# aconverse/ffmpeg-heaac

Measured on AMD Instinct MI355X. Metric: HE-AAC frames/s (batched), higher is better.
Workload: dtype f32; 1 GPU; HE-AACv2 stereo 48 kHz, 256 k-frame batch; frames_per_gpu=262144, pcm=f32, bytes_per_frame=85284, parallelism=frames sharded by index, no collective

## Files before the change

### ffmpeg-heaac_amd/__init__.py

```python
import ctypes as C
import os

import numpy as np

_HERE = os.path.dirname(os.path.abspath(__file__))
PRODUCT_LIB_PATH = os.path.join(_HERE, "libheaac_amd.so")
LIB_PATH = os.environ.get("HEAAC_LIB_PATH") or PRODUCT_LIB_PATH
LIB_OVERRIDDEN = os.path.realpath(LIB_PATH) != os.path.realpath(PRODUCT_LIB_PATH)

ONLY_LONG_SEQUENCE, LONG_START_SEQUENCE, EIGHT_SHORT_SEQUENCE, LONG_STOP_SEQUENCE = 0, 1, 2, 3
CFG_LC_MONO, CFG_LC_STEREO, CFG_HEV1, CFG_HEV2, CFG_HEV1_MONO = 0, 1, 2, 3, 4
PCM_F32, PCM_S16, PCM_S16_SSE2 = 0, 1, 2
ADD_BIAS = 385.0

ST_SAVED, ST_SBR, ST_SYNTH, ST_PS = 512, 1972, 1152, 4500
STATE_WORDS = {
    CFG_LC_MONO: ST_SAVED,
    CFG_LC_STEREO: 2 * ST_SAVED,
    CFG_HEV1: 2 * ST_SAVED + 2 * ST_SBR + 2 * ST_SYNTH,
    CFG_HEV1_MONO: ST_SAVED + ST_SBR + ST_SYNTH,
    CFG_HEV2: ST_SAVED + ST_SBR + 2 * ST_SYNTH + ST_PS,
}
CORE_CH = {CFG_LC_MONO: 1, CFG_LC_STEREO: 2, CFG_HEV1: 2, CFG_HEV2: 1, CFG_HEV1_MONO: 1}
OUT_CH = {CFG_LC_MONO: 1, CFG_LC_STEREO: 2, CFG_HEV1: 2, CFG_HEV2: 2, CFG_HEV1_MONO: 1}
OUT_LEN = {CFG_LC_MONO: 1024, CFG_LC_STEREO: 1024, CFG_HEV1: 2048, CFG_HEV2: 2048, CFG_HEV1_MONO: 2048}

ALGO_BYTES = {CFG_LC_STEREO: 24584, CFG_HEV1: 83976, CFG_HEV2: 85284}

ICS_DT = np.dtype([("window_sequence", "u1", (2,)), ("use_kb_window", "u1", (2,))])
SBR_HDR_DT = np.dtype([
    ("k0", "u1"), ("k2", "u1"), ("kx", "u1"), ("m", "u1"),
    ("n", "u1", (2,)), ("n_q", "u1"), ("n_lim", "u1"),
    ("n_master", "u1"), ("num_patches", "u1"), ("bs_limiter_gains", "u1"),
    ("bs_interpol_freq", "u1"), ("bs_smoothing_mode", "u1"), ("bs_amp_res_header", "u1"),
    ("pad0", "u1", (2,)),
    ("patch_num_subbands", "u1", (6,)), ("patch_start_subband", "u1", (6,)),
    ("f_tablenoise", "u1", (6,)), ("pad1", "u1", (2,)),
    ("f_tablelow", "u1", (28,)), ("f_tablehigh", "u1", (52,)), ("f_tablelim", "u1", (32,)),
    ("map_hi", "u1", (64,)), ("map_lo", "u1", (64,)), ("map_nq", "u1", (64,)),
    ("map_lim", "u1", (64,)), ("map_mid", "u1", (64,)), ("map_src", "u1", (64,)),
])
SBR_CH_DT = np.dtype([
    ("bs_num_env", "u1"), ("bs_num_noise", "u1"), ("bs_amp_res", "u1"), ("bs_add_harmonic_flag", "u1"),
    ("bs_freq_res", "u1", (8,)), ("t_env", "u1", (8,)), ("t_q", "u1", (3,)),
    ("t_env_num_env_old", "u1"), ("e_a", "i1", (2,)),
    ("bs_invf_mode", "u1", (2, 5)), ("bs_add_harmonic", "u1", (48,)),
# ... 1121 lines not shown
```

### ffmpeg-heaac_amd/csrc/capi.hip

```cpp
#include <hip/hip_runtime.h>
#include <stdint.h>
#include <stdlib.h>
#include <string.h>
#include "heaac_dsp.h"
#include "heaac_debug.h"
#include "heaac_parse.h"
#include "parse_core.h"
#include "sbr_core.h"
#include "tables.h"
#include "kernels.h"
#include "host_common.h"

#define HE_MAX_LANES 4
#define HE_ZERO_BYTES (2 * 38 * 64 * 4)
struct HeaacDevice {
    int device;
    float *d_tab;
    uint16_t *d_rev;
    HeaacParseTables *d_ptab;
    HeaacSbrParseTables *d_stab;
    void *d_work;
    unsigned *d_queue;
    unsigned char *d_aux;
    size_t work_bytes;
    size_t max_frames;
    size_t chunk;
    int sets;
    hipStream_t lane[HE_MAX_LANES];
    hipEvent_t fork, join[HE_MAX_LANES];
    int lanes;
    hipStream_t owner;
    hipEvent_t done;
    int owner_valid, done_recorded;
};

static int he_claim(HeaacDevice *d, hipStream_t s, bool *capturing)
{
// ... 88 lines not shown
    *out = NULL;
    int count = 0;
    if (hipGetDeviceCount(&count) != hipSuccess || count <= 0)
        return HEAAC_ERR_NODEVICE;
    HeaacDevice *d = (HeaacDevice *)calloc(1, sizeof(*d));
    if (!d) return HEAAC_ERR_NOMEM;
    if (hipGetDevice(&d->device) != hipSuccess) { free(d); return HEAAC_ERR_HIP; }
    hipDeviceProp_t prop;
    if (hipGetDeviceProperties(&prop, d->device) != hipSuccess ||
        strncmp(prop.gcnArchName, "gfx950", 6) != 0) {
        free(d);
        return HEAAC_ERR_NODEVICE;
    }
    HeaacHostTables *t = (HeaacHostTables *)malloc(sizeof(*t));
    if (!t) { free(d); return HEAAC_ERR_NOMEM; }
    heaac_build_tables(t);
    d->max_frames = max_frames;
    d->work_bytes = heaac_device_workspace_bytes(max_frames);
    d->chunk = he_chunk_frames(max_frames);
    d->sets = (int)he_sets(max_frames);
    int rc = HEAAC_OK;
    if (hipMalloc((void **)&d->d_tab, sizeof(t->f)) != hipSuccess ||
        hipMalloc((void **)&d->d_rev, sizeof(t->rev)) != hipSuccess ||
        hipMalloc((void **)&d->d_queue, 64 * HE_MAX_LANES) != hipSuccess ||
        hipMalloc((void **)&d->d_aux, HE_ZERO_BYTES + 2 * (size_t)(d->sets > 0 ? d->sets : 1) * (d->chunk ? d->chunk : 1)) != hipSuccess ||
        hipMalloc((void **)&d->d_ptab, sizeof(HeaacParseTables)) != hipSuccess ||
        hipMalloc((void **)&d->d_stab, sizeof(HeaacSbrParseTables)) != hipSuccess ||
        (d->work_bytes && hipMalloc(&d->d_work, d->work_bytes) != hipSuccess))
        rc = HEAAC_ERR_NOMEM;
    const HeaacParseTables *pt = heaac_parse_tables();
    if (rc == HEAAC_OK && (!pt || hipMemcpy(d->d_ptab, pt, sizeof(*pt), hipMemcpyHostToDevice) != hipSuccess))
        rc = HEAAC_ERR_HIP;
    const HeaacSbrParseTables *spt = heaac_sbr_parse_tables();
    if (rc == HEAAC_OK && (!spt || hipMemcpy(d->d_stab, spt, sizeof(*spt), hipMemcpyHostToDevice) != hipSuccess))
        rc = HEAAC_ERR_HIP;
    if (rc == HEAAC_OK &&
        (hipMemset(d->d_aux, 0, HE_ZERO_BYTES) != hipSuccess ||
         hipMemcpy(d->d_tab, t->f, sizeof(t->f), hipMemcpyHostToDevice) != hipSuccess ||
         hipMemcpy(d->d_rev, t->rev, sizeof(t->rev), hipMemcpyHostToDevice) != hipSuccess))
        rc = HEAAC_ERR_HIP;
    free(t);
    d->lanes = HE_LANES;
    if (rc == HEAAC_OK && (hipEventCreateWithFlags(&d->fork, hipEventDisableTiming) != hipSuccess ||
                           hipEventCreateWithFlags(&d->done, hipEventDisableTiming) != hipSuccess))
        rc = HEAAC_ERR_HIP;
    for (int k = 0; k < d->lanes && rc == HEAAC_OK; k++)
        if (hipEventCreateWithFlags(&d->join[k], hipEventDisableTiming) != hipSuccess ||
            hipStreamCreateWithFlags(&d->lane[k], hipStreamNonBlocking) != hipSuccess)
            rc = HEAAC_ERR_HIP;
    if (rc != HEAAC_OK) {
        heaac_device_destroy(d);
        return rc;
    }
    *out = d;
    return HEAAC_OK;
}

extern "C" void heaac_device_destroy(HeaacDevice *d)
{
    if (!d) return;
    if (d->d_tab) (void)hipFree(d->d_tab);
// ... 235 lines not shown
    const HeaacCfgShape shape = heaac_cfg_shape(cfg);
    const size_t ncore = shape.ncore, words = shape.words;
    const size_t pcm_bytes = (size_t)shape.nout * ((flags & HEAAC_HE_DOWNSAMPLED) ? 1024 : 2048) *
                             (pcm_format == HEAAC_PCM_F32_PLANAR ? 4 : 2);
    const size_t set_floats = dev->chunk * (WS_W_FLOATS + WS_X_FLOATS);
    const size_t per_chunk = dev->chunk / T;
    const unsigned hdrs = (unsigned)(n_hdr > 0xffffu ? 0x10000u : n_hdr);
    bool capturing = false;
    const int claim = he_claim(dev, s, &capturing);
    if (claim != HEAAC_OK) return claim;
    const bool lanes = n_streams > per_chunk && dev->sets > 1;
    const int nl = lanes ? dev->sets : 1;
    int rc = HEAAC_OK;
    int forked = 0;
    if (lanes) {
        if (hipEventRecord(dev->fork, s) != hipSuccess) rc = HEAAC_ERR_HIP;
        for (int k = 0; k < nl && rc == HEAAC_OK; k++) {
            if (hipStreamWaitEvent(dev->lane[k], dev->fork, 0) != hipSuccess) rc = HEAAC_ERR_HIP;
            else forked = k + 1;
        }
    }
    HeaacHeLaunch a = {};
    a.d_tab = dev->d_tab; a.d_rev = dev->d_rev; a.cfg = cfg; a.flags = flags; a.d_hdr = d_hdr; a.n_hdr = hdrs;
    a.pcm_format = pcm_format; a.d_zero = (const float *)dev->d_aux; a.T = T;
    size_t c = 0;
    for (size_t s0 = 0; s0 < n_streams && rc == HEAAC_OK; s0 += per_chunk, c++) {
        const size_t f0 = s0 * T;
        const int k = (int)(c % nl);
        a.n_streams = n_streams - s0 < per_chunk ? n_streams - s0 : per_chunk;
        a.d_coeffs = d_coeffs + f0 * ncore * 1024; a.d_ics = d_ics + f0 * ncore; a.d_sbr = d_sbr + f0;
        a.d_ps = d_ps ? d_ps + f0 : NULL; a.d_hold = d_hold ? d_hold + f0 : NULL;
        a.d_state_in = d_state_in + s0 * words; a.d_state_out = d_state_out + s0 * words;
        a.d_pcm = (char *)d_pcm + f0 * pcm_bytes;
        a.d_ws_W = (float *)dev->d_work + k * set_floats; a.d_ws_X = a.d_ws_W + dev->chunk * WS_W_FLOATS;
        a.d_queue = dev->d_queue + 16 * k; a.d_xtop = dev->d_aux + HE_ZERO_BYTES + 2 * (size_t)k * dev->chunk;
        a.s = lanes ? dev->lane[k] : s;
        rc = heaac_launch_he(&a);
    }
    if (lanes) {
        for (int k = 0; k < forked; k++)
            if (hipEventRecord(dev->join[k], dev->lane[k]) != hipSuccess ||
                hipStreamWaitEvent(s, dev->join[k], 0) != hipSuccess)
                rc = rc == HEAAC_OK ? HEAAC_ERR_HIP : rc;
    }
    return he_release(dev, s, capturing, rc);
}

extern "C" int heaac_he_decode_batch_ex(HeaacDevice *dev, int cfg, int flags,
                                     const float *d_coeffs, const HeaacIcs *d_ics,
                                     const HeaacSbrFrame *d_sbr,
                                     const HeaacSbrHeader *d_hdr, size_t n_hdr,
                                     const HeaacPsFrame *d_ps,
                                     const float *d_state_in, float *d_state_out,
                                     void *d_pcm, int pcm_format,
                                     size_t n, void *stream)
{
    if (!dev || !he_cfg_ok(cfg) || !pcm_format_ok(pcm_format) || (flags & ~HEAAC_HE_DOWNSAMPLED))
        return HEAAC_ERR_ARG;
// ... 105 lines not shown
    if (!dev || channels < 1 || channels > HEAAC_MAX_PCM_PLANES || len <= 0 || (len & 3) ||
        (pcm_format != HEAAC_PCM_S16_INTERLEAVED && pcm_format != HEAAC_PCM_S16_INTERLEAVED_SSE2))
        return HEAAC_ERR_ARG;
    if (n == 0) return HEAAC_OK;
    if (!planes || !d_out) return HEAAC_ERR_ARG;
    for (int c = 0; c < channels; c++)
        if (!planes[c].d_base || ((uintptr_t)planes[c].d_base & 15) || (planes[c].frame_stride & 3)) return HEAAC_ERR_ARG;
    return heaac_launch_interleave(channels, planes, len, pcm_format, d_out, n, (hipStream_t)stream);
}

extern "C" int heaac_debug_workspace(HeaacDevice *dev, float **d_W, float **d_X, size_t *chunk)
{
    if (!dev) return HEAAC_ERR_ARG;
    if (d_W) *d_W = (float *)dev->d_work;
    if (d_X) *d_X = (float *)dev->d_work + dev->chunk * WS_W_FLOATS;
    if (chunk) *chunk = dev->chunk;
    return HEAAC_OK;
}

extern "C" int heaac_debug_xbands(HeaacDevice *dev, unsigned char *host_out, size_t n_frames)
{
    if (!dev || !host_out || n_frames > (size_t)(dev->sets > 0 ? dev->sets : 1) * dev->chunk) return HEAAC_ERR_ARG;
    if (hipDeviceSynchronize() != hipSuccess) return HEAAC_ERR_HIP;
    return hipMemcpy(host_out, dev->d_aux + HE_ZERO_BYTES, 2 * n_frames, hipMemcpyDeviceToHost) == hipSuccess
               ? HEAAC_OK : HEAAC_ERR_HIP;
}

size_t heaac_device_max_frames_per_stream(const HeaacDevice *dev) { return dev ? dev->chunk : 0; }

extern "C" const float *heaac_device_tables(HeaacDevice *dev, const uint16_t **rev)
{
    if (rev) *rev = dev->d_rev;
    return dev->d_tab;
}
```

### ffmpeg-heaac_amd/csrc/k_common.h

```cpp
#pragma once
#include <hip/hip_runtime.h>
#include "heaac_dsp.h"
#include <stdint.h>
#include <type_traits>
#include "tables.h"

#define WAVE 64

__device__ __forceinline__ void wave_sync()
{
    __builtin_amdgcn_fence(__ATOMIC_RELEASE, "wavefront");
    __builtin_amdgcn_wave_barrier();
    __builtin_amdgcn_fence(__ATOMIC_ACQUIRE, "wavefront");
}

typedef float v2f __attribute__((ext_vector_type(2)));

__device__ __forceinline__ const uint8_t *hold_mask() { return nullptr; }
__device__ __forceinline__ const uint8_t *hold_mask(const uint8_t *p) { return p; }

#define HE_X_CHANNEL (38 * 64 * 2)

template <int ST_AUX>
struct GBufT {
// ... 55 lines not shown
        qoff = waves * Q;
        pos = 0;
        cur = wave * Q;
        unsigned t = 0;
        if (lane == 0) t = atomicAdd(queue, Q);
        base1 = qoff + (unsigned long long)__builtin_amdgcn_readfirstlane(t);
        nxt = Q > 1 ? cur + 1 : base1;
        vt = 0;
    }
    __device__ __forceinline__ void request(int lane)
    {
        if (pos == 0) { vt = 0; if (lane == 0) vt = atomicAdd(queue, Q); }
    }
    __device__ __forceinline__ void advance()
    {
        cur = nxt;
        if (pos + 1 < Q) {
            pos++;
        } else {
            pos = 0;
            base1 = qoff + (unsigned long long)__builtin_amdgcn_readfirstlane(vt);
        }
        nxt = pos + 1 < Q ? cur + 1 : base1;
    }
};

struct NoHook {
    __device__ __forceinline__ void operator()() const {}
    __device__ __forceinline__ void operator()(int) const {}
};

__device__ __forceinline__ unsigned lds_addr(const void *p)
{
    return __builtin_amdgcn_readfirstlane((unsigned)reinterpret_cast<uintptr_t>(p));
}
#define L2_TOUCH_STRIDE 128
__device__ __forceinline__ void l2_touch(const void *base, unsigned bytes, int lane, unsigned dump)
{
    for (unsigned o = 0; o < bytes; o += WAVE * L2_TOUCH_STRIDE) {
        unsigned off = o + (unsigned)lane * L2_TOUCH_STRIDE;
        off = off < bytes ? off : bytes - 4;
        const char *p = reinterpret_cast<const char *>(base) + off;
        unsigned keep;
        asm volatile("s_mov_b32 %0, m0\n\ts_mov_b32 m0, %2\n\ts_nop 0\n\t"
                     "global_load_lds_dword %1, off\n\ts_mov_b32 m0, %0"
                     : "=&s"(keep) : "v"(p), "s"(dump) : "memory");
// ... 236 lines not shown
```

### ffmpeg-heaac_amd/csrc/k_he.hip

```cpp
#include <type_traits>
#include "k_core.h"
#include "k_core2.h"
#include "kernels.h"
#include "host_common.h"

#include "k_hf.h"

#define ANA_WAVES 8
#define ANA_POOL  3456

struct AnaLds {
    CoreLds core;
    float qmf_ds[320];
    float rot[64];
    float pool[ANA_WAVES][ANA_POOL];
};

__device__ __forceinline__ void qmf_analysis_wave(const float *qmf_ds, const float *rot,
                                                  const float *c16, const float *c32,
                                                  const float *x, float *u, float *g_W, int lane)
{
    {
        const int k = lane;
        const float w0 = qmf_ds[k], w1 = qmf_ds[k + 64], w2 = qmf_ds[k + 128],
// ... 238 lines not shown
        int xb = 64;
        hf_channel(S, s_noise, sbr, g_hdr, n_hdr, ch, g_W + u * 2048,
                   g_state_in + f * state_words + off, g_state_out + f * state_words + off, lane,
                   [&](int i, float re, float im) {
                       if (i == 0 && g_xtop) {
                           const int top16 = (S.h.kx + S.h.m + 15) & ~15;
                           const int t_old = S.c[ch].t_env_num_env_old;
                           const bool zero = 2 * t_old - 32 <= 0 || (int)sbr->kx_old + (int)sbr->m_old <= top16;
                           xb = __builtin_amdgcn_readfirstlane(zero && top16 < 64 ? top16 : 64);
                           if (lane == 0 && xb != 64) g_xtop[f * 2 + ch] = (unsigned char)xb;
                       }
                       if (lane < xb) __builtin_nontemporal_store(v2f{re, im}, Xc + i * 64 + lane);
                   });
      }
        feed.advance();
    }
}

#define SYN_WAVES 6
#define VB_STRIDE 129
#define VB_ROWS   41

#define SYN_WAVES_F32 7
struct SynWave {
    __attribute__((aligned(16))) float vb[VB_ROWS * VB_STRIDE + 3];
};
template <int NW>
struct SynLdsT {
    float win[640];
    float rot[64];
    float c16[8], c32[12];
    SynWave w[NW];
};
typedef SynLdsT<SYN_WAVES> SynLds;

#ifdef HEAAC_STAMPS
#define SSTAMP(i) TL_STAMP(i, (i) == 0)
#else
#define SSTAMP(i) do {} while (0)
#endif

__device__ __forceinline__ float lane_xor1(float v)
{
    return __int_as_float(__builtin_amdgcn_update_dpp(0, __float_as_int(v), 0xB1, 0xF, 0xF, false));
}

struct SynIn {
    float x[64];
    float h[18];
};

#define SYN_STAGE_STRIDE 68
typedef float f32x4 __attribute__((ext_vector_type(4)));
__device__ __forceinline__ f32x4 syn_ld4(const f32x4 *p) { return __builtin_nontemporal_load(p); }
__device__ __forceinline__ float syn_ld1(const float *p) { return __builtin_nontemporal_load(p); }
template <class T>
__device__ __forceinline__ void syn_st(T *p, T v) { __builtin_nontemporal_store(v, p); }
__device__ __forceinline__ void syn_load_ring(const float *v_in, int lane, SynIn &d)
{
#pragma unroll
    for (int r = 0; r < 18; r++) d.h[r] = syn_ld1(v_in + lane + 64 * r);
}
template <bool PLANES, bool RING = true>
__device__ __forceinline__ void syn_load(const float *X0, const float *X1, const float *v_in, int lane, SynIn &d)
{
    const f32x4 *p0 = reinterpret_cast<const f32x4 *>(X0), *p1 = reinterpret_cast<const f32x4 *>(X1);
#pragma unroll
    for (int q = 0; q < 16; q++) {
        const f32x4 t = PLANES ? syn_ld4(q < 8 ? p0 + q * 64 + lane : p1 + (q - 8) * 64 + lane)
                               : syn_ld4(p0 + q * 64 + lane);
        d.x[4 * q] = t.x; d.x[4 * q + 1] = t.y; d.x[4 * q + 2] = t.z; d.x[4 * q + 3] = t.w;
    }
    if constexpr (RING) syn_load_ring(v_in, lane, d);
}

template <bool PLANES, class SL>
__device__ __forceinline__ void syn_rows(const SL &S, SynWave &w, const SynIn &d, int lane)
{
    float x[64];
    {
        float4 *st = reinterpret_cast<float4 *>(w.vb);
        if constexpr (PLANES) {
#pragma unroll
            for (int q = 0; q < 16; q++) {
                const int row = (q >> 3) * 32 + 4 * (q & 7) + (lane >> 4);
                st[(row * SYN_STAGE_STRIDE >> 2) + (lane & 15)] = make_float4(d.x[4 * q], d.x[4 * q + 1], d.x[4 * q + 2], d.x[4 * q + 3]);
            }
        } else {
            float2 *st2 = reinterpret_cast<float2 *>(w.vb);
#pragma unroll
            for (int q = 0; q < 16; q++) {
                const int slot = 2 * q + (lane >> 5), pi = lane & 31;
                st2[(slot * SYN_STAGE_STRIDE >> 1) + pi] = make_float2(d.x[4 * q], d.x[4 * q + 2]);
                st2[((32 + slot) * SYN_STAGE_STRIDE >> 1) + pi] = make_float2(d.x[4 * q + 1], d.x[4 * q + 3]);
            }
        }
        wave_sync();
        const int mine = (lane & 1) * 32 + (lane >> 1);
#pragma unroll
        for (int q = 0; q < 16; q++) {
            const float4 t = st[(mine * SYN_STAGE_STRIDE >> 2) + q];
            x[4 * q] = t.x; x[4 * q + 1] = t.y; x[4 * q + 2] = t.z; x[4 * q + 3] = t.w;
        }
        wave_sync();
    }
    SSTAMP(1);
#pragma unroll
    for (int r = 0; r < 18; r++)
        w.vb[(32 + (r >> 1)) * VB_STRIDE + (r & 1) * 64 + lane] = d.h[r];
    const int i = lane >> 1, part = lane & 1;
    const unsigned flip = (unsigned)part << 31;
    float o[64];
    imdct128_reg([&](int j) -> float {
                     return (j & 1) ? __uint_as_float(__float_as_uint(x[j]) ^ flip) : x[j];
                 }, o, S.rot, S.c16, S.c32);
    SSTAMP(2);
    float *vs = w.vb + (31 - i) * VB_STRIDE + 64 * part;
    const unsigned neg = (unsigned)(part ^ 1) << 31;
#pragma unroll
    for (int n = 0; n < 64; n++) {
        const float mine = __uint_as_float(__float_as_uint(o[63 - n]) ^ neg);
        vs[n] = lane_xor1(o[n]) + mine;
    }
}

template <int UNROLL = 1, class SL, class Emit>
__device__ __forceinline__ void syn_poly(const SL &S, const SynWave &w, float scale, float bias, int lane, Emit emit)
{
    SSTAMP(3);
    const int n = lane;
    float wt[10];
#pragma unroll
    for (int j = 0; j < 10; j++) wt[j] = S.win[64 * j + n];
    const bool scale_and_bias = scale != 1.0f || bias != 0.0f;
#pragma unroll UNROLL
    for (int i = 0; i < 32; i += 2) {
        const float *va = w.vb + (31 - i) * VB_STRIDE + n, *vb = va - VB_STRIDE;
        v2f acc = v2f{va[0], vb[0]} * bc(wt[0]) + v2f{0.0f, 0.0f};
        acc = v2f{va[1 * VB_STRIDE + 64], vb[1 * VB_STRIDE + 64]} * bc(wt[1]) + acc;
        acc = v2f{va[2 * VB_STRIDE],      vb[2 * VB_STRIDE]}      * bc(wt[2]) + acc;
        acc = v2f{va[3 * VB_STRIDE + 64], vb[3 * VB_STRIDE + 64]} * bc(wt[3]) + acc;
        acc = v2f{va[4 * VB_STRIDE],      vb[4 * VB_STRIDE]}      * bc(wt[4]) + acc;
        acc = v2f{va[5 * VB_STRIDE + 64], vb[5 * VB_STRIDE + 64]} * bc(wt[5]) + acc;
        acc = v2f{va[6 * VB_STRIDE],      vb[6 * VB_STRIDE]}      * bc(wt[6]) + acc;
        acc = v2f{va[7 * VB_STRIDE + 64], vb[7 * VB_STRIDE + 64]} * bc(wt[7]) + acc;
        acc = v2f{va[8 * VB_STRIDE],      vb[8 * VB_STRIDE]}      * bc(wt[8]) + acc;
        acc = v2f{va[9 * VB_STRIDE + 64], vb[9 * VB_STRIDE + 64]} * bc(wt[9]) + acc;
        if (scale_and_bias) acc = acc * bc(scale) + bc(bias);
        emit(i, n, acc.x);
        emit(i + 1, n, acc.y);
    }
    SSTAMP(4);
}

__device__ __forceinline__ void syn_hist_out(const SynWave &w, float *v_out, int lane)
{
#pragma unroll
    for (int r = 0; r < 18; r++)
        syn_st(v_out + lane + 64 * r, w.vb[(r >> 1) * VB_STRIDE + (r & 1) * 64 + lane]);
}

template <int UNROLL = 1, class SL, class Emit>
__device__ __forceinline__ void synth_channel(const SL &S, SynWave &w, const float *X0, const float *X1,
                                              const float *v_in, float *v_out,
                                              float scale, float bias, int lane, Emit emit)
{
    SSTAMP(0);
    SynIn d;
    syn_load<true>(X0, X1, v_in, lane, d);
    syn_rows<true>(S, w, d, lane);
    wave_sync();
    syn_poly<UNROLL>(S, w, scale, bias, lane, emit);
    syn_hist_out(w, v_out, lane);
    wave_sync();
    SSTAMP(5);
}

template <int FMT>
__global__ __launch_bounds__(SYN_WAVES_F32 * WAVE)
void k_synth(const float *__restrict__ g_tab, const float *g_X,
             const float *g_state_in, float *g_state_out, int state_words, int off_syn0,
             int nout, void *__restrict__ g_pcm, float scale, float bias,
             unsigned long long n_frames, unsigned long long pcm_frame0, unsigned *g_queue,
             const unsigned char *__restrict__ g_xtop, const float *__restrict__ g_zero)
{
    constexpr int NW = SYN_WAVES_F32;
    __shared__ SynLdsT<NW> S;
    for (int i = threadIdx.x; i < 640; i += blockDim.x) S.win[i] = g_tab[TB_QMF_US + i];
    if (threadIdx.x < 64) S.rot[threadIdx.x] = g_tab[TB_ROT128S + threadIdx.x];
    if (threadIdx.x < 5) S.c16[threadIdx.x] = g_tab[TB_COS16 + threadIdx.x];
    if (threadIdx.x < 9) S.c32[threadIdx.x] = g_tab[TB_COS32 + threadIdx.x];
    __syncthreads();
    const int wave = __builtin_amdgcn_readfirstlane(threadIdx.x / WAVE), lane = threadIdx.x % WAVE;
    SynWave &w = S.w[wave];
    auto load_unit = [&](unsigned long long f, int ch, SynIn &d) {
        const int xt = __builtin_amdgcn_readfirstlane((int)g_xtop[f * 2 + ch]);
        const float *X0 = (lane & 31) * 2 < xt ? g_X + (f * 2 + ch) * HE_X_CHANNEL : g_zero;
        syn_load<false>(X0, nullptr, g_state_in + f * state_words + off_syn0 + ch * HEAAC_ST_SYNTH, lane, d);
    };
    FrameFeed<2> feed;
    feed.init((unsigned long long)blockIdx.x * NW + wave, (unsigned long long)gridDim.x * NW, g_queue, lane);
    SynIn cur;
    if (feed.cur < n_frames) load_unit(feed.cur, 0, cur);
    while (feed.cur < n_frames) {
        const unsigned long long f = feed.cur, f1 = feed.nxt;
        feed.request(lane);
        float *st_out = g_state_out + f * state_words + off_syn0;
        auto channel = [&](int ch, auto emit) {
            SSTAMP(0);
            syn_rows<false>(S, w, cur, lane);
            wave_sync();
            if (ch + 1 < nout) load_unit(f, ch + 1, cur);
            else if (f1 < n_frames) load_unit(f1, 0, cur);
            syn_poly<1>(S, w, scale, bias, lane, emit);
            syn_hist_out(w, st_out + ch * HEAAC_ST_SYNTH, lane);
            wave_sync();
            SSTAMP(5);
        };
        if (FMT == HEAAC_PCM_F32_PLANAR) {
            for (int ch = 0; ch < nout; ch++) {
                float *o = reinterpret_cast<float *>(g_pcm) + ((pcm_frame0 + f) * nout + ch) * 2048;
                channel(ch, [&](int i, int n, float v) { syn_st(o + 64 * i + n, v); });
            }
        } else {
            int16_t *o = reinterpret_cast<int16_t *>(g_pcm) + (pcm_frame0 + f) * 2048 * nout;
            for (int ch = 0; ch < nout; ch++)
                channel(ch, [&](int i, int n, float v) {
                    o[(64 * i + n) * nout + ch] = (int16_t)pcm_int16<FMT>(v);
                });
        }
        feed.advance();
    }
}

template <int FMT, class... Hold>
__global__ __launch_bounds__(SYN_WAVES_F32 * WAVE)
void k_synth_streams(const float *__restrict__ g_tab, const float *g_X,
                     const float *g_state_in, float *g_state_out, int state_words, int off_syn0,
                     int nout, void *__restrict__ g_pcm, float scale, float bias,
                     unsigned long long n_streams, unsigned T, unsigned *g_queue,
                     const unsigned char *__restrict__ g_xtop, const float *__restrict__ g_zero, Hold... hold)
{
    constexpr bool HOLD = sizeof...(Hold) != 0;
    constexpr int NW = SYN_WAVES_F32;
    __shared__ SynLdsT<NW> S;
    for (int i = threadIdx.x; i < 640; i += blockDim.x) S.win[i] = g_tab[TB_QMF_US + i];
    if (threadIdx.x < 64) S.rot[threadIdx.x] = g_tab[TB_ROT128S + threadIdx.x];
    if (threadIdx.x < 5) S.c16[threadIdx.x] = g_tab[TB_COS16 + threadIdx.x];
    if (threadIdx.x < 9) S.c32[threadIdx.x] = g_tab[TB_COS32 + threadIdx.x];
    __syncthreads();
    const int wave = __builtin_amdgcn_readfirstlane(threadIdx.x / WAVE), lane = threadIdx.x % WAVE;
    SynWave &w = S.w[wave];
    const unsigned long long n_chains = n_streams * nout;
    auto load_x = [&](unsigned long long st, unsigned t, int ch, SynIn &d) {
        const unsigned long long u = (unsigned long long)t * n_streams + st;
        const int xt = __builtin_amdgcn_readfirstlane((int)g_xtop[u * 2 + ch]);
        const float *X0 = (lane & 31) * 2 < xt ? g_X + (u * 2 + ch) * HE_X_CHANNEL : g_zero;
        syn_load<false, false>(X0, nullptr, nullptr, lane, d);
    };
    auto load_chain = [&](unsigned long long c, SynIn &d) {
        const unsigned long long st = c / nout;
        const int ch = (int)(c - st * nout);
        load_x(st, 0, ch, d);
        syn_load_ring(g_state_in + st * state_words + off_syn0 + ch * HEAAC_ST_SYNTH, lane, d);
    };
    FrameFeed<2> feed;
    feed.init((unsigned long long)blockIdx.x * NW + wave, (unsigned long long)gridDim.x * NW, g_queue, lane);
    SynIn cur;
    if (feed.cur < n_chains) load_chain(feed.cur, cur);
    while (feed.cur < n_chains) {
        const unsigned long long c = feed.cur, c1 = feed.nxt;
        feed.request(lane);
        const unsigned long long st = c / nout;
        const int ch = (int)(c - st * nout);
        for (unsigned t = 0; t < T; t++) {
            const bool last = t + 1 == T;
            [[maybe_unused]] bool held = false;
            if constexpr (HOLD) {
                held = __builtin_amdgcn_readfirstlane((int)hold_mask(hold...)[st * T + t]) != 0;
                if (held && last) {
                    float *v_out = g_state_out + st * state_words + off_syn0 + ch * HEAAC_ST_SYNTH;
#pragma unroll
                    for (int q = 0; q < 18; q++) syn_st(v_out + lane + 64 * q, cur.h[q]);
                }
            }
            if (!HOLD || !held) {
                syn_rows<false>(S, w, cur, lane);
                wave_sync();
            }
            if (!last) load_x(st, t + 1, ch, cur);
            else if (c1 < n_chains) load_chain(c1, cur);
            const unsigned long long r = st * T + t;
            if constexpr (HOLD) {
                if (held) {
                    if constexpr (FMT == HEAAC_PCM_F32_PLANAR) {
                        float *o = reinterpret_cast<float *>(g_pcm) + (r * nout + ch) * 2048;
#pragma nounroll
                        for (int q = lane; q < 2048; q += WAVE) o[q] = 0.0f;
                    } else {
                        int16_t *o = reinterpret_cast<int16_t *>(g_pcm) + r * 2048 * nout;
#pragma nounroll
                        for (int q = lane; q < 2048; q += WAVE) o[q * nout + ch] = 0;
                    }
                    continue;
                }
            }
            if constexpr (FMT == HEAAC_PCM_F32_PLANAR) {
                float *o = reinterpret_cast<float *>(g_pcm) + (r * nout + ch) * 2048;
                syn_poly<1>(S, w, scale, bias, lane, [&](int i, int n, float v) { syn_st(o + 64 * i + n, v); });
            } else {
                int16_t *o = reinterpret_cast<int16_t *>(g_pcm) + r * 2048 * nout;
                syn_poly<1>(S, w, scale, bias, lane,
                            [&](int i, int n, float v) { o[(64 * i + n) * nout + ch] = (int16_t)pcm_int16<FMT>(v); });
            }
            if (!last) {
#pragma unroll
                for (int q = 0; q < 18; q++) cur.h[q] = w.vb[(q >> 1) * VB_STRIDE + (q & 1) * 64 + lane];
            } else {
                syn_hist_out(w, g_state_out + st * state_words + off_syn0 + ch * HEAAC_ST_SYNTH, lane);
            }
            wave_sync();
        }
        feed.advance();
    }
}

__global__ __launch_bounds__(ANA_WAVES * WAVE)
void k_qmf_analysis(const float *__restrict__ g_tab, const float *__restrict__ g_in,
                    const float *g_xh_in, float *g_xh_out, float *__restrict__ g_W, float scale,
                    unsigned long long n)
{
    __shared__ float qmf_ds[320];
    __shared__ float rot[64];
    __shared__ float c16[8], c32[12];
    __shared__ float pool[ANA_WAVES][ANA_POOL];
    for (int i = threadIdx.x; i < 320; i += blockDim.x) qmf_ds[i] = g_tab[TB_QMF_DS + i];
    if (threadIdx.x < 64) rot[threadIdx.x] = g_tab[TB_ROT128A + threadIdx.x];
    if (threadIdx.x < 5) c16[threadIdx.x] = g_tab[TB_COS16 + threadIdx.x];
    if (threadIdx.x < 9) c32[threadIdx.x] = g_tab[TB_COS32 + threadIdx.x];
    __syncthreads();
    const int wave = __builtin_amdgcn_readfirstlane(threadIdx.x / WAVE), lane = threadIdx.x % WAVE;
    float *p = pool[wave];
    for (unsigned long long u = (unsigned long long)blockIdx.x * ANA_WAVES + wave; u < n;
         u += (unsigned long long)gridDim.x * ANA_WAVES) {
        float *x = p + 2080;
        for (int i = lane; i < 288; i += WAVE) x[i] = g_xh_in[u * 288 + i];
// ... 239 lines not shown
    const HeaacCfgShape c = heaac_cfg_shape(a->cfg);
    if (!c.he) return HEAAC_ERR_ARG;
    if (!a->n_streams || !a->T) return HEAAC_OK;
    const bool strided = a->T > 1 || a->d_hold;
    const int ncore = c.ncore, nout = c.nout, words = (int)c.words;
    const unsigned long long S = a->n_streams, T = a->T, units = S * ncore;
    const float *const d_tab = a->d_tab;
    float *const state_out = a->d_state_out;
    hipStream_t s = a->s;
    const bool simd = a->pcm_format == HEAAC_PCM_S16_INTERLEAVED_SSE2;
    const float sf_scale = simd ? -1.0f / 1024.0f : HEAAC_SF_SCALE;
    HIP_OK(hipMemsetAsync(a->d_xtop, 64, 2 * S * T, s));
    const float *state_in = a->d_state_in;
    if (a->d_hold && state_in != state_out) {
        HIP_OK(hipMemcpyAsync(state_out, state_in, S * (size_t)words * sizeof(float), hipMemcpyDeviceToDevice, s));
        state_in = state_out;
    }
    for (size_t t = 0; t < T; t++) {
        const float *st_in = t ? state_out : state_in;
        float *W = a->d_ws_W + t * units * 2048;
        float *X = a->d_ws_X + t * S * 2 * HE_X_CHANNEL;
        unsigned char *xtop = a->d_xtop + 2 * t * S;
        const uint8_t *hold = a->d_hold ? a->d_hold + t : nullptr;
        HIP_OK(hipMemsetAsync(a->d_queue, 0, 64, s));
        with_strided_hold(strided, hold, [&](auto st, auto... m) {
            k_core_ana<st()><<<persistent_grid((units + 1) / 2, CA_WAVES), CA_WAVES * WAVE, 0, s>>>(
                d_tab, a->d_rev, a->d_coeffs + t * ncore * 1024, a->d_ics + t * ncore, st_in, state_out, words, ncore, 0,
                c.off_sbr, W, 1 / (-1024 * sf_scale), units, T, m...);
        });
        if (a->cfg == HEAAC_CFG_HEV2) {
            int rc = heaac_launch_hfps(a, t, st_in, W, X);
            if (rc != HEAAC_OK) return rc;
            rc = heaac_launch_ps(a, t, st_in, X);
            if (rc != HEAAC_OK) return rc;
        } else {
            with_strided_hold(strided, hold, [&](auto st, auto... m) {
                k_hfadj<st()><<<persistent_grid((units + 1) / 2, HF_WAVES), HF_WAVES * WAVE, 0, s>>>(
                    d_tab, a->d_sbr + t, a->d_hdr, a->n_hdr, W, st_in, state_out, words, ncore, c.off_sbr, X, units,
                    a->d_queue + 1, xtop, T, m...);
            });
        }
    }
    const float scale = -1024 * sf_scale, bias = simd ? 0.0f : HEAAC_ADD_BIAS;
    const bool ds = a->flags & HEAAC_HE_DOWNSAMPLED;
    const int waves = ds ? DS_WAVES : SYN_WAVES_F32;
    const dim3 g = persistent_grid(strided ? S * nout : S, waves), b(waves * WAVE);
    const bool known = with_pcm_format(a->pcm_format, [&](auto fmt) {
        if (!strided && ds)
            k_synth_ds<fmt()><<<g, b, 0, s>>>(d_tab, a->d_ws_X, state_in, state_out, words, c.off_syn, nout, a->d_pcm,
                                              scale, bias, S);
        else if (!strided)
            k_synth<fmt()><<<g, b, 0, s>>>(d_tab, a->d_ws_X, state_in, state_out, words, c.off_syn, nout, a->d_pcm, scale,
                                           bias, S, 0ull, a->d_queue + 2, a->d_xtop, a->d_zero);
        else if (ds)
            with_hold(a->d_hold, [&](auto... m) {
                k_synth_ds_streams<fmt()><<<g, b, 0, s>>>(d_tab, a->d_ws_X, state_in, state_out, words, c.off_syn, nout,
                                                          a->d_pcm, scale, bias, S, (unsigned)T, m...);
            });
        else
            with_hold(a->d_hold, [&](auto... m) {
                k_synth_streams<fmt()><<<g, b, 0, s>>>(d_tab, a->d_ws_X, state_in, state_out, words, c.off_syn, nout, a->d_pcm,
                                                       scale, bias, S, (unsigned)T, a->d_queue + 2, a->d_xtop, a->d_zero,
                                                       m...);
            });
    });
    if (!known) return HEAAC_ERR_ARG;
    return hipGetLastError() == hipSuccess ? HEAAC_OK : HEAAC_ERR_HIP;
}

extern "C" int heaac_launch_qmf_analysis(const float *d_tab, const float *d_in, const float *d_xh_in,
                                         float *d_xh_out, float *d_W, float scale, size_t n, hipStream_t s)
{
    if (!n) return HEAAC_OK;
    hipLaunchKernelGGL(k_qmf_analysis, persistent_grid(n, ANA_WAVES), dim3(ANA_WAVES * WAVE), 0, s,
                       d_tab, d_in, d_xh_in, d_xh_out, d_W, scale, (unsigned long long)n);
    return hipGetLastError() == hipSuccess ? HEAAC_OK : HEAAC_ERR_HIP;
}

extern "C" int heaac_launch_qmf_synthesis(const float *d_tab, const float *d_X, const float *d_v_in,
                                          float *d_v_out, float *d_out, float scale, float bias,
                                          size_t n, hipStream_t s)
{
    if (!n) return HEAAC_OK;
    hipLaunchKernelGGL(k_qmf_synthesis, persistent_grid(n, SYN_WAVES), dim3(SYN_WAVES * WAVE), 0, s,
                       d_tab, d_X, d_v_in, d_v_out, d_out, scale, bias, (unsigned long long)n);
    return hipGetLastError() == hipSuccess ? HEAAC_OK : HEAAC_ERR_HIP;
// ... 21 lines not shown
```

### ffmpeg-heaac_amd/csrc/kernels.h

```cpp
#pragma once
#include <hip/hip_runtime.h>
#include <stddef.h>
#include <stdint.h>
#include "heaac_dsp.h"

extern "C" {
int heaac_launch_lc(const float *d_tab, const uint16_t *d_rev, int channels,
                    const float *d_coeffs, const HeaacIcs *d_ics,
                    const float *d_state_in, float *d_state_out,
                    void *d_pcm, int pcm_format, size_t n_streams, size_t frames_per_stream,
                    const uint8_t *d_hold, hipStream_t s);

int heaac_launch_imdct_half(const float *d_tab, const uint16_t *d_rev, int which,
                            float *d_out, const float *d_in, size_t n, hipStream_t s);

int heaac_launch_couple(int channels, float *d_pcm, const float *d_cce, const HeaacCoupling *d_cpl,
                        int16_t *d_s16, size_t n, hipStream_t s);

int heaac_launch_interleave(int channels, const HeaacPlaneRef *planes, int len, int pcm_format, int16_t *d_out,
                            size_t n, hipStream_t s);

struct HeaacHeLaunch {
    const float *d_tab;
    const uint16_t *d_rev;
    int cfg, flags;
    const HeaacSbrHeader *d_hdr;
    unsigned n_hdr;
    const float *d_coeffs;
    const HeaacIcs *d_ics;
    const HeaacSbrFrame *d_sbr;
    const HeaacPsFrame *d_ps;
    const float *d_state_in;
    float *d_state_out;
    void *d_pcm;
    int pcm_format;
    float *d_ws_W, *d_ws_X;
    unsigned *d_queue;
    unsigned char *d_xtop;
    const float *d_zero;
    size_t n_streams, T;
    const uint8_t *d_hold;
    hipStream_t s;
};
int heaac_launch_he(const struct HeaacHeLaunch *a);

int heaac_launch_hfps(const struct HeaacHeLaunch *a, size_t t, const float *st_in, const float *W, float *X);
int heaac_launch_ps(const struct HeaacHeLaunch *a, size_t t, const float *st_in, float *X);

int heaac_launch_qmf_analysis(const float *d_tab, const float *d_in, const float *d_xh_in,
                              float *d_xh_out, float *d_W, float scale, size_t n, hipStream_t s);

int heaac_launch_qmf_synthesis(const float *d_tab, const float *d_X, const float *d_v_in,
                               float *d_v_out, float *d_out, float scale, float bias,
                               size_t n, hipStream_t s);

int heaac_launch_qmf_synthesis_ds(const float *d_tab, const float *d_X, const float *d_v_in,
                                  float *d_v_out, float *d_out, float scale, float bias,
                                  size_t n, hipStream_t s);

int heaac_launch_spectral_tools(int channels, float *d_coeffs, const HeaacToolsFrame *d_tools,
                                const int *d_rng_in, int *d_rng_out,
                                const HeaacPredictorState *d_pred_in, HeaacPredictorState *d_pred_out,
                                int stages, const HeaacCceFrame *d_cce, const float *d_cce_coeffs, int n_cce,
                                size_t n, hipStream_t s);

int heaac_launch_spectral_tools_streams(int channels, float *d_coeffs, const HeaacToolsFrame *d_tools,
                                        const int *d_rng_in, int *d_rng_out,
// ... 39 lines not shown
```

Measured before the change: 26.34 million frames/s.

## Spread synthesis work queue over eight atomic heads and vectorize ring history I/O

Replaces the single atomic counter feeding the persistent synthesis kernels with eight separate queue heads. Each block starts on its own head and moves to the next when that head's partition is exhausted, which is meant to reduce atomic contention. The synthesis ring history is now loaded and stored as float4/float2 vectors with a matching LDS layout. The zero buffer for inactive X lanes is dropped in favour of register zero-fill with predicated loads. These changes add queue-memory sizing changes and more complex work-stealing logic.

```diff
diff --git a/ffmpeg-heaac_amd/__init__.py b/ffmpeg-heaac_amd/__init__.py
--- a/ffmpeg-heaac_amd/__init__.py
+++ b/ffmpeg-heaac_amd/__init__.py
@@ -22,6 +22,8 @@
     CFG_HEV2: ST_SAVED + ST_SBR + 2 * ST_SYNTH + ST_PS,
 }
 CORE_CH = {CFG_LC_MONO: 1, CFG_LC_STEREO: 2, CFG_HEV1: 2, CFG_HEV2: 1, CFG_HEV1_MONO: 1}
+SYNTH_WAVES_PER_BLOCK, PERSISTENT_BLOCKS, SYNTH_FEED_CHUNK, SYNTH_FEED_HEADS = 7, 256, 2, 8
+SYNTH_FEED_WAVES = SYNTH_WAVES_PER_BLOCK * PERSISTENT_BLOCKS
 OUT_CH = {CFG_LC_MONO: 1, CFG_LC_STEREO: 2, CFG_HEV1: 2, CFG_HEV2: 2, CFG_HEV1_MONO: 1}
 OUT_LEN = {CFG_LC_MONO: 1024, CFG_LC_STEREO: 1024, CFG_HEV1: 2048, CFG_HEV2: 2048, CFG_HEV1_MONO: 2048}
 
diff --git a/ffmpeg-heaac_amd/csrc/capi.hip b/ffmpeg-heaac_amd/csrc/capi.hip
--- a/ffmpeg-heaac_amd/csrc/capi.hip
+++ b/ffmpeg-heaac_amd/csrc/capi.hip
@@ -12,7 +12,6 @@
 #include "host_common.h"
 
 #define HE_MAX_LANES 4
-#define HE_ZERO_BYTES (2 * 38 * 64 * 4)
 struct HeaacDevice {
     int device;
     float *d_tab;
@@ -147,8 +146,8 @@
     int rc = HEAAC_OK;
     if (hipMalloc((void **)&d->d_tab, sizeof(t->f)) != hipSuccess ||
         hipMalloc((void **)&d->d_rev, sizeof(t->rev)) != hipSuccess ||
-        hipMalloc((void **)&d->d_queue, 64 * HE_MAX_LANES) != hipSuccess ||
-        hipMalloc((void **)&d->d_aux, HE_ZERO_BYTES + 2 * (size_t)(d->sets > 0 ? d->sets : 1) * (d->chunk ? d->chunk : 1)) != hipSuccess ||
+        hipMalloc((void **)&d->d_queue, HE_QUEUE_WORDS * sizeof(unsigned) * HE_MAX_LANES) != hipSuccess ||
+        hipMalloc((void **)&d->d_aux, 2 * (size_t)(d->sets > 0 ? d->sets : 1) * (d->chunk ? d->chunk : 1)) != hipSuccess ||
         hipMalloc((void **)&d->d_ptab, sizeof(HeaacParseTables)) != hipSuccess ||
         hipMalloc((void **)&d->d_stab, sizeof(HeaacSbrParseTables)) != hipSuccess ||
         (d->work_bytes && hipMalloc(&d->d_work, d->work_bytes) != hipSuccess))
@@ -160,8 +159,7 @@
     if (rc == HEAAC_OK && (!spt || hipMemcpy(d->d_stab, spt, sizeof(*spt), hipMemcpyHostToDevice) != hipSuccess))
         rc = HEAAC_ERR_HIP;
     if (rc == HEAAC_OK &&
-        (hipMemset(d->d_aux, 0, HE_ZERO_BYTES) != hipSuccess ||
-         hipMemcpy(d->d_tab, t->f, sizeof(t->f), hipMemcpyHostToDevice) != hipSuccess ||
+        (hipMemcpy(d->d_tab, t->f, sizeof(t->f), hipMemcpyHostToDevice) != hipSuccess ||
          hipMemcpy(d->d_rev, t->rev, sizeof(t->rev), hipMemcpyHostToDevice) != hipSuccess))
         rc = HEAAC_ERR_HIP;
     free(t);
@@ -443,7 +441,7 @@
     }
     HeaacHeLaunch a = {};
     a.d_tab = dev->d_tab; a.d_rev = dev->d_rev; a.cfg = cfg; a.flags = flags; a.d_hdr = d_hdr; a.n_hdr = hdrs;
-    a.pcm_format = pcm_format; a.d_zero = (const float *)dev->d_aux; a.T = T;
+    a.pcm_format = pcm_format; a.T = T;
     size_t c = 0;
     for (size_t s0 = 0; s0 < n_streams && rc == HEAAC_OK; s0 += per_chunk, c++) {
         const size_t f0 = s0 * T;
@@ -454,7 +452,7 @@
         a.d_state_in = d_state_in + s0 * words; a.d_state_out = d_state_out + s0 * words;
         a.d_pcm = (char *)d_pcm + f0 * pcm_bytes;
         a.d_ws_W = (float *)dev->d_work + k * set_floats; a.d_ws_X = a.d_ws_W + dev->chunk * WS_W_FLOATS;
-        a.d_queue = dev->d_queue + 16 * k; a.d_xtop = dev->d_aux + HE_ZERO_BYTES + 2 * (size_t)k * dev->chunk;
+        a.d_queue = dev->d_queue + HE_QUEUE_WORDS * k; a.d_xtop = dev->d_aux + 2 * (size_t)k * dev->chunk;
         a.s = lanes ? dev->lane[k] : s;
         rc = heaac_launch_he(&a);
     }
@@ -606,7 +604,7 @@
 {
     if (!dev || !host_out || n_frames > (size_t)(dev->sets > 0 ? dev->sets : 1) * dev->chunk) return HEAAC_ERR_ARG;
     if (hipDeviceSynchronize() != hipSuccess) return HEAAC_ERR_HIP;
-    return hipMemcpy(host_out, dev->d_aux + HE_ZERO_BYTES, 2 * n_frames, hipMemcpyDeviceToHost) == hipSuccess
+    return hipMemcpy(host_out, dev->d_aux, 2 * n_frames, hipMemcpyDeviceToHost) == hipSuccess
                ? HEAAC_OK : HEAAC_ERR_HIP;
 }
 
diff --git a/ffmpeg-heaac_amd/csrc/k_common.h b/ffmpeg-heaac_amd/csrc/k_common.h
--- a/ffmpeg-heaac_amd/csrc/k_common.h
+++ b/ffmpeg-heaac_amd/csrc/k_common.h
@@ -101,6 +101,71 @@
             base1 = qoff + (unsigned long long)__builtin_amdgcn_readfirstlane(vt);
         }
         nxt = pos + 1 < Q ? cur + 1 : base1;
+    }
+};
+
+#define FEED_HEADS 8
+#define FEED_HEAD_WORDS 16
+template <unsigned Q, unsigned NQ = FEED_HEADS>
+struct FrameFeedHeads {
+    unsigned long long cur, nxt;
+    unsigned long long base1;
+    unsigned long long qoff, part, n;
+    unsigned *queue;
+    unsigned head, left;
+    unsigned pos;
+    unsigned vt;
+
+    __device__ __forceinline__ unsigned draw(int lane) const
+    {
+        unsigned t = 0;
+        if (lane == 0) t = atomicAdd(queue + head * FEED_HEAD_WORDS, Q);
+        return t;
+    }
+    __device__ __forceinline__ unsigned long long take(unsigned t, int lane)
+    {
+        while (left) {
+            const unsigned long long f = qoff + head * part + t;
+            if (t < part && f < n) return f;
+            do {
+                if (--left == 0) return n;
+                head = (head + 1) % NQ;
+            } while (qoff + head * part >= n);
+            t = __builtin_amdgcn_readfirstlane(draw(lane));
+        }
+        return n;
+    }
+    __device__ __forceinline__ void init(unsigned long long wave, unsigned long long waves, unsigned home,
+                                         unsigned long long frames, unsigned *q, int lane)
+    {
+        queue = q;
+        n = frames;
+        qoff = waves * Q;
+        const unsigned long long rest = n > qoff ? n - qoff : 0;
+        part = (rest + NQ * Q - 1) / (NQ * Q) * Q;
+        head = home % NQ;
+        left = rest ? NQ : 0;
+        pos = 0;
+        cur = wave * Q;
+        base1 = left ? take(__builtin_amdgcn_readfirstlane(draw(lane)), lane) : n;
+        nxt = Q > 1 && cur + 1 < n ? cur + 1 : base1;
+        vt = 0;
+    }
+    __device__ __forceinline__ void request(int lane)
+    {
+        if (pos == 0 && left) vt = draw(lane);
+    }
+    __device__ __forceinline__ void advance(int lane)
+    {
+        const bool inside = pos + 1 < Q && cur + 1 < n;
+        cur = nxt;
+        if (inside) {
+            pos++;
+        } else {
+            pos = 0;
+            base1 = take(__builtin_amdgcn_readfirstlane(vt), lane);
+        }
+        nxt = pos + 1 < Q && cur + 1 < n ? cur + 1 : base1;
     }
 };
 
diff --git a/ffmpeg-heaac_amd/csrc/k_he.hip b/ffmpeg-heaac_amd/csrc/k_he.hip
--- a/ffmpeg-heaac_amd/csrc/k_he.hip
+++ b/ffmpeg-heaac_amd/csrc/k_he.hip
@@ -284,6 +284,10 @@
 #define VB_ROWS   41
 
 #define SYN_WAVES_F32 7
+#ifndef SYN_FEED_CHUNK
+#define SYN_FEED_CHUNK 2
+#endif
+static_assert(HE_QUEUE_WORDS == HE_QUEUE_SYNTH + FEED_HEADS * FEED_HEAD_WORDS, "kernels.h sizes the synthesis feed's heads");
 struct SynWave {
     __attribute__((aligned(16))) float vb[VB_ROWS * VB_STRIDE + 3];
 };
@@ -307,33 +311,64 @@
     return __int_as_float(__builtin_amdgcn_update_dpp(0, __float_as_int(v), 0xB1, 0xF, 0xF, false));
 }
 
+typedef float f32x4 __attribute__((ext_vector_type(4)));
 struct SynIn {
-    float x[64];
+    f32x4 x[16];
     float h[18];
 };
 
 #define SYN_STAGE_STRIDE 68
-typedef float f32x4 __attribute__((ext_vector_type(4)));
 __device__ __forceinline__ f32x4 syn_ld4(const f32x4 *p) { return __builtin_nontemporal_load(p); }
-__device__ __forceinline__ float syn_ld1(const float *p) { return __builtin_nontemporal_load(p); }
 template <class T>
 __device__ __forceinline__ void syn_st(T *p, T v) { __builtin_nontemporal_store(v, p); }
+typedef float f32x2 __attribute__((ext_vector_type(2)));
 __device__ __forceinline__ void syn_load_ring(const float *v_in, int lane, SynIn &d)
 {
 #pragma unroll
-    for (int r = 0; r < 18; r++) d.h[r] = syn_ld1(v_in + lane + 64 * r);
+    for (int q = 0; q < 4; q++) {
+        const f32x4 t = syn_ld4(reinterpret_cast<const f32x4 *>(v_in) + q * 64 + lane);
+        d.h[4 * q] = t.x; d.h[4 * q + 1] = t.y; d.h[4 * q + 2] = t.z; d.h[4 * q + 3] = t.w;
+    }
+    const f32x2 t = __builtin_nontemporal_load(reinterpret_cast<const f32x2 *>(v_in + 1024) + lane);
+    d.h[16] = t.x; d.h[17] = t.y;
+}
+__device__ __forceinline__ void syn_ring_put(SynWave &w, int row0, const float *h, int lane)
+{
+    float *v = w.vb + (row0 + (lane >> 5)) * VB_STRIDE + 4 * (lane & 31);
+#pragma unroll
+    for (int r = 0; r < 16; r++) v[2 * (r >> 2) * VB_STRIDE + (r & 3)] = h[r];
+    w.vb[(row0 + 8) * VB_STRIDE + 2 * lane] = h[16];
+    w.vb[(row0 + 8) * VB_STRIDE + 2 * lane + 1] = h[17];
+}
+__device__ __forceinline__ void syn_ring_get(const SynWave &w, int row0, float *h, int lane)
+{
+    const float *v = w.vb + (row0 + (lane >> 5)) * VB_STRIDE + 4 * (lane & 31);
+#pragma unroll
+    for (int r = 0; r < 16; r++) h[r] = v[2 * (r >> 2) * VB_STRIDE + (r & 3)];
+    h[16] = w.vb[(row0 + 8) * VB_STRIDE + 2 * lane];
+    h[17] = w.vb[(row0 + 8) * VB_STRIDE + 2 * lane + 1];
+}
+__device__ __forceinline__ void syn_store_ring(float *v_out, const float *h, int lane)
+{
+#pragma unroll
+    for (int q = 0; q < 4; q++)
+        syn_st(reinterpret_cast<f32x4 *>(v_out) + q * 64 + lane, f32x4{h[4 * q], h[4 * q + 1], h[4 * q + 2], h[4 * q + 3]});
+    syn_st(reinterpret_cast<f32x2 *>(v_out + 1024) + lane, f32x2{h[16], h[17]});
 }
 template <bool PLANES, bool RING = true>
 __device__ __forceinline__ void syn_load(const float *X0, const float *X1, const float *v_in, int lane, SynIn &d)
 {
     const f32x4 *p0 = reinterpret_cast<const f32x4 *>(X0), *p1 = reinterpret_cast<const f32x4 *>(X1);
 #pragma unroll
-    for (int q = 0; q < 16; q++) {
-        const f32x4 t = PLANES ? syn_ld4(q < 8 ? p0 + q * 64 + lane : p1 + (q - 8) * 64 + lane)
-                               : syn_ld4(p0 + q * 64 + lane);
-        d.x[4 * q] = t.x; d.x[4 * q + 1] = t.y; d.x[4 * q + 2] = t.z; d.x[4 * q + 3] = t.w;
-    }
+    for (int q = 0; q < 16; q++)
+        d.x[q] = PLANES ? syn_ld4(q < 8 ? p0 + q * 64 + lane : p1 + (q - 8) * 64 + lane) : syn_ld4(p0 + q * 64 + lane);
     if constexpr (RING) syn_load_ring(v_in, lane, d);
+}
+__device__ __forceinline__ void syn_load_stored(const float *X0, int xt, int lane, SynIn &d)
+{
+#pragma unroll
+    for (int q = 0; q < 16; q++) d.x[q] = f32x4{0.0f, 0.0f, 0.0f, 0.0f};
+    if ((lane & 31) * 2 < xt) syn_load<false, false>(X0, nullptr, nullptr, opaque(lane), d);
 }
 
 template <bool PLANES, class SL>
@@ -346,15 +381,14 @@
 #pragma unroll
             for (int q = 0; q < 16; q++) {
                 const int row = (q >> 3) * 32 + 4 * (q & 7) + (lane >> 4);
-                st[(row * SYN_STAGE_STRIDE >> 2) + (lane & 15)] = make_float4(d.x[4 * q], d.x[4 * q + 1], d.x[4 * q + 2], d.x[4 * q + 3]);
+                st[(row * SYN_STAGE_STRIDE >> 2) + (lane & 15)] = make_float4(d.x[q].x, d.x[q].y, d.x[q].z, d.x[q].w);
             }
         } else {
-            float2 *st2 = reinterpret_cast<float2 *>(w.vb);
+            float2 *st2 = reinterpret_cast<float2 *>(w.vb) + opaque((lane >> 5) * (SYN_STAGE_STRIDE >> 1) + (lane & 31));
 #pragma unroll
             for (int q = 0; q < 16; q++) {
-                const int slot = 2 * q + (lane >> 5), pi = lane & 31;
-                st2[(slot * SYN_STAGE_STRIDE >> 1) + pi] = make_float2(d.x[4 * q], d.x[4 * q + 2]);
-                st2[((32 + slot) * SYN_STAGE_STRIDE >> 1) + pi] = make_float2(d.x[4 * q + 1], d.x[4 * q + 3]);
+                st2[q * SYN_STAGE_STRIDE] = make_float2(d.x[q].x, d.x[q].z);
+                st2[(16 + q) * SYN_STAGE_STRIDE] = make_float2(d.x[q].y, d.x[q].w);
             }
         }
         wave_sync();
@@ -367,9 +401,7 @@
         wave_sync();
     }
     SSTAMP(1);
-#pragma unroll
-    for (int r = 0; r < 18; r++)
-        w.vb[(32 + (r >> 1)) * VB_STRIDE + (r & 1) * 64 + lane] = d.h[r];
+    syn_ring_put(w, 32, d.h, lane);
     const int i = lane >> 1, part = lane & 1;
     const unsigned flip = (unsigned)part << 31;
     float o[64];
@@ -377,7 +409,7 @@
                      return (j & 1) ? __uint_as_float(__float_as_uint(x[j]) ^ flip) : x[j];
                  }, o, S.rot, S.c16, S.c32);
     SSTAMP(2);
-    float *vs = w.vb + (31 - i) * VB_STRIDE + 64 * part;
+    float *vs = w.vb + opaque((31 - i) * VB_STRIDE + 64 * part);
     const unsigned neg = (unsigned)(part ^ 1) << 31;
 #pragma unroll
     for (int n = 0; n < 64; n++) {
@@ -417,9 +449,9 @@
 
 __device__ __forceinline__ void syn_hist_out(const SynWave &w, float *v_out, int lane)
 {
-#pragma unroll
-    for (int r = 0; r < 18; r++)
-        syn_st(v_out + lane + 64 * r, w.vb[(r >> 1) * VB_STRIDE + (r & 1) * 64 + lane]);
+    float h[18];
+    syn_ring_get(w, 0, h, lane);
+    syn_store_ring(v_out, h, lane);
 }
 
 template <int UNROLL = 1, class SL, class Emit>
@@ -444,7 +476,7 @@
              const float *g_state_in, float *g_state_out, int state_words, int off_syn0,
              int nout, void *__restrict__ g_pcm, float scale, float bias,
              unsigned long long n_frames, unsigned long long pcm_frame0, unsigned *g_queue,
-             const unsigned char *__restrict__ g_xtop, const float *__restrict__ g_zero)
+             const unsigned char *__restrict__ g_xtop)
 {
     constexpr int NW = SYN_WAVES_F32;
     __shared__ SynLdsT<NW> S;
@@ -457,11 +489,12 @@
     SynWave &w = S.w[wave];
     auto load_unit = [&](unsigned long long f, int ch, SynIn &d) {
         const int xt = __builtin_amdgcn_readfirstlane((int)g_xtop[f * 2 + ch]);
-        const float *X0 = (lane & 31) * 2 < xt ? g_X + (f * 2 + ch) * HE_X_CHANNEL : g_zero;
-        syn_load<false>(X0, nullptr, g_state_in + f * state_words + off_syn0 + ch * HEAAC_ST_SYNTH, lane, d);
+        syn_load_stored(g_X + (f * 2 + ch) * HE_X_CHANNEL, xt, lane, d);
+        syn_load_ring(g_state_in + f * state_words + off_syn0 + ch * HEAAC_ST_SYNTH, lane, d);
     };
-    FrameFeed<2> feed;
-    feed.init((unsigned long long)blockIdx.x * NW + wave, (unsigned long long)gridDim.x * NW, g_queue, lane);
+    FrameFeedHeads<SYN_FEED_CHUNK> feed;
+    feed.init((unsigned long long)blockIdx.x * NW + wave, (unsigned long long)gridDim.x * NW, blockIdx.x, n_frames, g_queue,
+              lane);
     SynIn cur;
     if (feed.cur < n_frames) load_unit(feed.cur, 0, cur);
     while (feed.cur < n_frames) {
@@ -491,7 +524,7 @@
                     o[(64 * i + n) * nout + ch] = (int16_t)pcm_int16<FMT>(v);
                 });
         }
-        feed.advance();
+        feed.advance(lane);
     }
 }
 
@@ -501,7 +534,7 @@
                      const float *g_state_in, float *g_state_out, int state_words, int off_syn0,
                      int nout, void *__restrict__ g_pcm, float scale, float bias,
                      unsigned long long n_streams, unsigned T, unsigned *g_queue,
-                     const unsigned char *__restrict__ g_xtop, const float *__restrict__ g_zero, Hold... hold)
+                     const unsigned char *__restrict__ g_xtop, Hold... hold)
 {
     constexpr bool HOLD = sizeof...(Hold) != 0;
     constexpr int NW = SYN_WAVES_F32;
@@ -517,8 +550,7 @@
     auto load_x = [&](unsigned long long st, unsigned t, int ch, SynIn &d) {
         const unsigned long long u = (unsigned long long)t * n_streams + st;
         const int xt = __builtin_amdgcn_readfirstlane((int)g_xtop[u * 2 + ch]);
-        const float *X0 = (lane & 31) * 2 < xt ? g_X + (u * 2 + ch) * HE_X_CHANNEL : g_zero;
-        syn_load<false, false>(X0, nullptr, nullptr, lane, d);
+        syn_load_stored(g_X + (u * 2 + ch) * HE_X_CHANNEL, xt, lane, d);
     };
     auto load_chain = [&](unsigned long long c, SynIn &d) {
         const unsigned long long st = c / nout;
@@ -526,8 +558,9 @@
         load_x(st, 0, ch, d);
         syn_load_ring(g_state_in + st * state_words + off_syn0 + ch * HEAAC_ST_SYNTH, lane, d);
     };
-    FrameFeed<2> feed;
-    feed.init((unsigned long long)blockIdx.x * NW + wave, (unsigned long long)gridDim.x * NW, g_queue, lane);
+    FrameFeedHeads<SYN_FEED_CHUNK> feed;
+    feed.init((unsigned long long)blockIdx.x * NW + wave, (unsigned long long)gridDim.x * NW, blockIdx.x, n_chains, g_queue,
+              lane);
     SynIn cur;
     if (feed.cur < n_chains) load_chain(feed.cur, cur);
     while (feed.cur < n_chains) {
@@ -542,8 +575,7 @@
                 held = __builtin_amdgcn_readfirstlane((int)hold_mask(hold...)[st * T + t]) != 0;
                 if (held && last) {
                     float *v_out = g_state_out + st * state_words + off_syn0 + ch * HEAAC_ST_SYNTH;
-#pragma unroll
-                    for (int q = 0; q < 18; q++) syn_st(v_out + lane + 64 * q, cur.h[q]);
+                    syn_store_ring(v_out, cur.h, lane);
                 }
             }
             if (!HOLD || !held) {
@@ -576,14 +608,13 @@
                             [&](int i, int n, float v) { o[(64 * i + n) * nout + ch] = (int16_t)pcm_int16<FMT>(v); });
             }
             if (!last) {
-#pragma unroll
-                for (int q = 0; q < 18; q++) cur.h[q] = w.vb[(q >> 1) * VB_STRIDE + (q & 1) * 64 + lane];
+                syn_ring_get(w, 0, cur.h, lane);
             } else {
                 syn_hist_out(w, g_state_out + st * state_words + off_syn0 + ch * HEAAC_ST_SYNTH, lane);
             }
             wave_sync();
         }
-        feed.advance();
+        feed.advance(lane);
     }
 }
 
@@ -869,7 +900,7 @@
         float *X = a->d_ws_X + t * S * 2 * HE_X_CHANNEL;
         unsigned char *xtop = a->d_xtop + 2 * t * S;
         const uint8_t *hold = a->d_hold ? a->d_hold + t : nullptr;
-        HIP_OK(hipMemsetAsync(a->d_queue, 0, 64, s));
+        HIP_OK(hipMemsetAsync(a->d_queue, 0, HE_QUEUE_WORDS * sizeof(unsigned), s));
         with_strided_hold(strided, hold, [&](auto st, auto... m) {
             k_core_ana<st()><<<persistent_grid((units + 1) / 2, CA_WAVES), CA_WAVES * WAVE, 0, s>>>(
                 d_tab, a->d_rev, a->d_coeffs + t * ncore * 1024, a->d_ics + t * ncore, st_in, state_out, words, ncore, 0,
@@ -898,7 +929,7 @@
                                               scale, bias, S);
         else if (!strided)
             k_synth<fmt()><<<g, b, 0, s>>>(d_tab, a->d_ws_X, state_in, state_out, words, c.off_syn, nout, a->d_pcm, scale,
-                                           bias, S, 0ull, a->d_queue + 2, a->d_xtop, a->d_zero);
+                                           bias, S, 0ull, a->d_queue + HE_QUEUE_SYNTH, a->d_xtop);
         else if (ds)
             with_hold(a->d_hold, [&](auto... m) {
                 k_synth_ds_streams<fmt()><<<g, b, 0, s>>>(d_tab, a->d_ws_X, state_in, state_out, words, c.off_syn, nout,
@@ -907,8 +938,7 @@
         else
             with_hold(a->d_hold, [&](auto... m) {
                 k_synth_streams<fmt()><<<g, b, 0, s>>>(d_tab, a->d_ws_X, state_in, state_out, words, c.off_syn, nout, a->d_pcm,
-                                                       scale, bias, S, (unsigned)T, a->d_queue + 2, a->d_xtop, a->d_zero,
-                                                       m...);
+                                                       scale, bias, S, (unsigned)T, a->d_queue + HE_QUEUE_SYNTH, a->d_xtop, m...);
             });
     });
     if (!known) return HEAAC_ERR_ARG;
diff --git a/ffmpeg-heaac_amd/csrc/kernels.h b/ffmpeg-heaac_amd/csrc/kernels.h
--- a/ffmpeg-heaac_amd/csrc/kernels.h
+++ b/ffmpeg-heaac_amd/csrc/kernels.h
@@ -37,12 +37,13 @@
     float *d_ws_W, *d_ws_X;
     unsigned *d_queue;
     unsigned char *d_xtop;
-    const float *d_zero;
     size_t n_streams, T;
     const uint8_t *d_hold;
     hipStream_t s;
 };
 int heaac_launch_he(const struct HeaacHeLaunch *a);
+#define HE_QUEUE_SYNTH 16
+#define HE_QUEUE_WORDS (HE_QUEUE_SYNTH + 8 * 16)
 
 int heaac_launch_hfps(const struct HeaacHeLaunch *a, size_t t, const float *st_in, const float *W, float *X);
 int heaac_launch_ps(const struct HeaacHeLaunch *a, size_t t, const float *st_in, float *X);
```

Measured after the change: 26.72 million frames/s (median of 6 runs). Within noise of the previous version (+1.4%).
